# eduardburlacu/DiTSep

Measured on AMD Instinct MI355X. Metric: separated utterances/sec @ N=30, 2-spk 4 s mixtures, higher is better.
Workload: dtype fp16 (fp16 MFMA operands, fp32 accumulate)

## Files before the change

ditsep_amd/csrc/common.h:

```cpp
#pragma once
#include <hip/hip_runtime.h>
#include <stdint.h>

typedef unsigned short op16_t;
typedef __attribute__((ext_vector_type(8))) unsigned short op16x8;
typedef __attribute__((ext_vector_type(4))) unsigned short op16x4;
typedef __attribute__((ext_vector_type(8))) __bf16 bf16x8;
typedef __attribute__((ext_vector_type(8))) _Float16 f16x8;
typedef __attribute__((ext_vector_type(4))) float f32x4;

#define DSN_WAVE 64

#define DSN_PL(planes, f16) ((planes) | ((f16) << 4))
#define PL_COUNT(pl) ((pl)&3)
#define PL_F16(pl) ((pl) >> 4)

enum { DSN_ACT_NONE = 0, DSN_ACT_ELU = 1, DSN_ACT_SNAKE = 2, DSN_ACT_SILU = 3 };
enum { DSN_F32_NONE = 0, DSN_F32_TANH = 1 };

__device__ __forceinline__ float dsn_elu(float v) { return v > 0.f ? v : expm1f(v); }
__device__ __forceinline__ float dsn_silu(float v) { return v / (1.f + __expf(-v)); }
__device__ __forceinline__ float dsn_snake(float v, float alpha, float inv_beta) {
  float s = __sinf(v * alpha);
  return v + inv_beta * s * s;
}

#define DSN_F16_MAX 65504.f
__device__ __forceinline__ float dsn_sat16(float v) {
  const float c = __builtin_amdgcn_fmed3f(v, -DSN_F16_MAX, DSN_F16_MAX);
  return v != v ? v : c;
}
__device__ __forceinline__ op16_t to_op16(float v, int f16) {
  return f16 ? __builtin_bit_cast(unsigned short, (_Float16)dsn_sat16(v)) : __builtin_bit_cast(unsigned short, (__bf16)v);
}
__device__ __forceinline__ float from_op16(op16_t u, int f16) {
  return f16 ? (float)__builtin_bit_cast(_Float16, u) : (float)__builtin_bit_cast(__bf16, u);
}
__device__ __forceinline__ void dsn_split(float v, op16_t& hi, op16_t& lo, int f16) {
  hi = to_op16(v, f16);
  lo = to_op16(v - from_op16(hi, f16), f16);
}

typedef __attribute__((ext_vector_type(8))) int i32x8;
#define DSN_FP8_MAX 448.f
__device__ __forceinline__ int dsn_mx_exp(float amax) {
  const unsigned u = __builtin_bit_cast(unsigned, amax * (1.f / DSN_FP8_MAX));
  const int k = (int)((u >> 23) & 0xffu) - 127 + ((u & 0x7fffffu) ? 1 : 0);
  return min(max(k, -126), 126);
}
__device__ __forceinline__ float dsn_pow2(int k) { return __builtin_bit_cast(float, (unsigned)(127 + k) << 23); }
__device__ __forceinline__ unsigned dsn_fp8x4(const f32x4& v) {
  float c[4];
#pragma unroll
  for (int r = 0; r < 4; ++r) {
    const float m = __builtin_amdgcn_fmed3f(v[r], -DSN_FP8_MAX, DSN_FP8_MAX);
    c[r] = v[r] != v[r] ? v[r] : m;
  }
  int w = __builtin_amdgcn_cvt_pk_fp8_f32(c[0], c[1], 0, false);
  w = __builtin_amdgcn_cvt_pk_fp8_f32(c[2], c[3], w, true);
  return (unsigned)w;
}
__device__ __forceinline__ f32x4 mfma_mx8(const op16x8& w_lo, const op16x8& w_hi, const op16x8& a_lo, const op16x8& a_hi,
                                          const f32x4& c, int sw, int sa) {
  typedef __attribute__((ext_vector_type(4))) int i32x4;
  const i32x4 wl = __builtin_bit_cast(i32x4, w_lo), wh = __builtin_bit_cast(i32x4, w_hi);
  const i32x4 al = __builtin_bit_cast(i32x4, a_lo), ah = __builtin_bit_cast(i32x4, a_hi);
  const i32x8 w = {wl[0], wl[1], wl[2], wl[3], wh[0], wh[1], wh[2], wh[3]};
  const i32x8 a = {al[0], al[1], al[2], al[3], ah[0], ah[1], ah[2], ah[3]};
  return __builtin_amdgcn_mfma_scale_f32_16x16x128_f8f6f4(w, a, c, 0, 0, 0, sw, 0, sa);
}

template <int F16>
__device__ __forceinline__ f32x4 mfma16(const op16x8& w, const op16x8& a, const f32x4& c) {
  if (F16)
    return __builtin_amdgcn_mfma_f32_16x16x32_f16(__builtin_bit_cast(f16x8, w), __builtin_bit_cast(f16x8, a), c, 0, 0, 0);
  else
    return __builtin_amdgcn_mfma_f32_16x16x32_bf16(__builtin_bit_cast(bf16x8, w), __builtin_bit_cast(bf16x8, a), c, 0, 0,
                                                   0);
}

__device__ __forceinline__ float wave_sum(float v) {
#pragma unroll
  for (int o = 32; o > 0; o >>= 1) v += __shfl_xor(v, o, 64);
  return v;
}
__device__ __forceinline__ float wave_max(float v) {
#pragma unroll
  for (int o = 32; o > 0; o >>= 1) v = fmaxf(v, __shfl_xor(v, o, 64));
  return v;
}

struct GnGeom {
  int G, cpg, qpg;
};
__host__ __device__ inline GnGeom gn_geom(int C) {
  const int G = C / 4 < 32 ? C / 4 : 32;
  return GnGeom{G, C / G, C / G / 4};
}
__host__ __device__ inline int gn_tpg(int G, int block) {
  int tpg = 1;
  while (tpg < 64 && G * tpg * 2 <= block) tpg *= 2;
  return tpg;
}
// ... 64 lines not shown
```

ditsep_amd/csrc/igemm.hip:

```cpp
#include "igemm.h"

#ifndef DSN_SETPRIO
#define DSN_SETPRIO 0
#endif

namespace {

constexpr int BM = 128, BN = 128, BK = 32;
constexpr int TILE_ELEMS = 128 * BK;

__device__ __forceinline__ int swz(int row, int chunk) { return chunk ^ ((-(row >> 2)) & 3); }

enum { EPI_STATS = 1, EPI_LNFOLD = 2, EPI_FP8OUT = 4 };
enum { LEAN_NO_DIT = 1, LEAN_NO_NCSN = 2, LEAN_SEEDED = 4 };

template <int NT, int MT>
__device__ __forceinline__ void seed_acc(const GemmDesc& d, f32x4 (&acc)[NT][MT], int mw0, int m_end, int nw0, int lane) {
  const int nq = (lane >> 4) * 4;
#pragma unroll
  for (int tm = 0; tm < MT; ++tm) {
    const int m = mw0 + tm * 16 + (lane & 15);
    const bool mok = m < m_end;
    const int b = mok ? m / d.rows_per_b : 0;
    const int j = mok ? m - b * d.rows_per_b : 0;
// ... 245 lines not shown
  if constexpr ((LEAN & LEAN_SEEDED) == 0 && BIAS_FIRST) {
    if (!f_swiglu) {
#pragma unroll
      for (int tn = 0; tn < NT; ++tn) {
        const int n = nw0 + tn * 16 + nq;
        gbias[tn] = (d.bias && n < d.N) ? *reinterpret_cast<const f32x4*>(d.bias + (n % d.bias_mod)) : f32x4{0.f, 0.f, 0.f, 0.f};
      }
#pragma unroll
      for (int tn = 0; tn < NT; ++tn) dsn_touch(gbias[tn]);
    }
  }
  float gmean[NT], gm2[NT];
#pragma unroll
  for (int tn = 0; tn < NT; ++tn) gmean[tn] = gm2[tn] = 0.f;
#pragma unroll
  for (int tm = 0; tm < MT; ++tm) {
    const int m = mw0 + tm * 16 + (lane & 15);
    if (m >= m_end) continue;
    const int b = m / d.rows_per_b;
    const int j = m - b * d.rows_per_b;
    const long row_rel = (long)j * d.out_row_elems + d.out_off;
    const long row_abs = (long)b * d.out_bstride + row_rel;
    if (!f_swiglu) {
      if (!ROPE_FIRST && f_rope) {
        const int section = nw0 / d.qkv_D;
        if (section < 2 && (nw0 & 63) == 0) {
          const int pos = m % d.rope_S;
          const f32x4 c0 = *reinterpret_cast<const f32x4*>(d.rope_cos + pos * 32 + nq);
          const f32x4 s0 = *reinterpret_cast<const f32x4*>(d.rope_sin + pos * 32 + nq);
          const f32x4 c1 = *reinterpret_cast<const f32x4*>(d.rope_cos + pos * 32 + 16 + nq);
          const f32x4 s1 = *reinterpret_cast<const f32x4*>(d.rope_sin + pos * 32 + 16 + nq);
          const f32x4 x0 = acc[0][tm], x1 = acc[1][tm];
          acc[0][tm] = x0 * c0 - x1 * s0;
          acc[1][tm] = x1 * c1 + x0 * s1;
        }
      }
#pragma unroll
      for (int tn = 0; tn < NT; ++tn) {
        const int n = nw0 + tn * 16 + nq;
        if (n >= d.N) continue;
        const long rel = row_rel + n;
        if (rel < 0 || rel >= d.out_limit) continue;
        const long off = row_abs + n;
        f32x4 v = acc[tn][tm];
        if constexpr ((LEAN & LEAN_SEEDED) == 0) {
          if constexpr (BIAS_FIRST) v += gbias[tn];
          else if (d.bias) v += *reinterpret_cast<const f32x4*>(d.bias + (n % d.bias_mod));
          if (f_qkv && n < d.qkv_D) v *= d.q_scale;
          if (f_bbias) v += *reinterpret_cast<const f32x4*>(d.bbias + (long)b * d.bbias_stride + n);
          if (d.resid)
            v += *reinterpret_cast<const f32x4*>(d.resid + (long)b * d.resid_bstride + (long)j * d.resid_row_elems +
                                                 d.resid_off + n);
        }
        v *= d.out_scale;
        if (f_gn) {
          const float mb = 0.25f * ((v[0] + v[1]) + (v[2] + v[3]));
          float m2b = 0.f;
#pragma unroll
          for (int r = 0; r < 4; ++r) {
            const float dl = v[r] - mb;
            m2b += dl * dl;
          }
          if (tm == 0) {
            gmean[tn] = mb;
            gm2[tn] = m2b;
          } else {
            const float dm = mb - gmean[tn];
            gmean[tn] += dm * (1.f / (float)(tm + 1));
            gm2[tn] += m2b + dm * dm * (4.f * (float)tm / (float)(tm + 1));
          }
        }
        if (d.out_f32) {
          f32x4 o = v;
          if (f_tanh) {
#pragma unroll
            for (int r = 0; r < 4; ++r) o[r] = tanhf(v[r]);
          }
          *reinterpret_cast<f32x4*>(d.out_f32 + off) = o;
        }
        if (d.out_planes) {
          f32x4 a = v;
          if (d.act == DSN_ACT_ELU) {
#pragma unroll
            for (int r = 0; r < 4; ++r) a[r] = dsn_elu(v[r]);
          } else if (d.act == DSN_ACT_SILU) {
#pragma unroll
            for (int r = 0; r < 4; ++r) a[r] = dsn_silu(v[r]);
          } else if (d.act == DSN_ACT_SNAKE) {
            const int ch = n % d.act_mod;
            const f32x4 al = *reinterpret_cast<const f32x4*>(d.act_a + ch);
            const f32x4 ib = *reinterpret_cast<const f32x4*>(d.act_b + ch);
#pragma unroll
            for (int r = 0; r < 4; ++r) a[r] = dsn_snake(v[r], al[r], ib[r]);
          }
          op16x4 hi, lo;
#pragma unroll
          for (int r = 0; r < 4; ++r) {
            op16_t h, l;
            dsn_split(a[r], h, l, F16);
            hi[r] = h;
            lo[r] = l;
          }
          *reinterpret_cast<op16x4*>(d.out_planes + off) = hi;
          if (P == 2) *reinterpret_cast<op16x4*>(d.out_planes + d.out_ps + off) = lo;
        }
      }
    } else if ((EPI & EPI_FP8OUT) && d.out_fp8) {
      static_assert(!(EPI & EPI_FP8OUT) || NT == 4, "fp8 SwiGLU epilogue expects 64 packed columns per wave");
      f32x4 h[2];
      float amax = 0.f;
#pragma unroll
      for (int tp = 0; tp < 2; ++tp) {
        const int np = nw0 + tp * 32;
        f32x4 val = acc[2 * tp][tm], gate = acc[2 * tp + 1][tm];
        if (d.bias && np < d.N) {
          val += *reinterpret_cast<const f32x4*>(d.bias + np + nq);
          gate += *reinterpret_cast<const f32x4*>(d.bias + np + 16 + nq);
        }
#pragma unroll
        for (int r = 0; r < 4; ++r) {
          h[tp][r] = val[r] * dsn_silu(gate[r]);
          amax = fmaxf(amax, fabsf(h[tp][r]));
        }
      }
      amax = fmaxf(amax, __shfl_xor(amax, 16, 64));
      amax = fmaxf(amax, __shfl_xor(amax, 32, 64));
      const int k = dsn_mx_exp(amax);
      const float inv = dsn_pow2(-k);
      if (nw0 < d.N) {
        const long orow = (long)m * (d.N >> 1);
#pragma unroll
        for (int tp = 0; tp < 2; ++tp)
          *reinterpret_cast<unsigned*>(d.out_fp8 + orow + (nw0 >> 1) + tp * 16 + nq) = dsn_fp8x4(h[tp] * inv);
        if ((lane >> 4) == 0) d.out_fp8_scale[(long)m * (d.N >> 6) + (nw0 >> 6)] = (unsigned char)(k + 127);
      }
    } else {
#pragma unroll
      for (int tp = 0; tp < NT / 2; ++tp) {
        const int np = nw0 + tp * 32;
        if (np >= d.N) continue;
        const int feat = (np >> 1) + nq;
        const long off = row_abs + feat;
        f32x4 val = acc[2 * tp][tm], gate = acc[2 * tp + 1][tm];
        if (d.bias) {
          val += *reinterpret_cast<const f32x4*>(d.bias + np + nq);
          gate += *reinterpret_cast<const f32x4*>(d.bias + np + 16 + nq);
        }
        op16x4 hi, lo;
#pragma unroll
        for (int r = 0; r < 4; ++r) {
          op16_t h, l;
          dsn_split(val[r] * dsn_silu(gate[r]), h, l, F16);
          hi[r] = h;
          lo[r] = l;
        }
        *reinterpret_cast<op16x4*>(d.out_planes + off) = hi;
        if (P == 2) *reinterpret_cast<op16x4*>(d.out_planes + d.out_ps + off) = lo;
      }
    }
  }
  if (f_gn && mw0 < m_end) {
    const int b = mw0 / d.rows_per_b;
    const int slice = (mw0 - b * d.rows_per_b) >> 6;
    const int S = d.rows_per_b >> 6;
#pragma unroll
    for (int tn = 0; tn < NT; ++tn) {
      float cnt = (float)(MT * 4);
// ... 1486 lines not shown
```

ditsep_amd/csrc/kernels.hip:

```cpp
#include "kernels.h"

namespace {

constexpr int TPB = 256;
inline int grid_for(long n, int per_block = TPB, int cap = 256 * 16) {
  long g = (n + per_block - 1) / per_block;
  return (int)(g < 1 ? 1 : (g > cap ? cap : g));
}

__device__ __forceinline__ void store_planes(op16_t* dst, long ps, int planes, long i, float v) {
  op16_t h, l;
  dsn_split(v, h, l, PL_F16(planes));
  dst[i] = h;
  if (PL_COUNT(planes) == 2) dst[ps + i] = l;
}

__global__ void pack_tokens_kernel(const float* __restrict__ s0, int C0, const float* __restrict__ s1, int C1,
                                   int B, int T, float* __restrict__ df, op16_t* __restrict__ dp, long ps,
                                   int planes) {
  const int C = C0 + C1;
  const long n = (long)B * T * C;
  for (long i = blockIdx.x * (long)blockDim.x + threadIdx.x; i < n; i += (long)gridDim.x * blockDim.x) {
    const int c = (int)(i % C);
    const long bt = i / C;
// ... 533 lines not shown
                                                             int L, int C, int apply_tanh) {
  constexpr int TILE = 256;
  extern __shared__ __attribute__((aligned(16))) float smem[];
  const int NJ = C / 32;
  f32x4* wl4 = reinterpret_cast<f32x4*>(smem);
  float* part = smem + KT * C;
  const int blocks_per_seq = (L + TILE - 1) / TILE;
  const int s = blockIdx.x / blocks_per_seq;
  const int l0 = (blockIdx.x - s * blocks_per_seq) * TILE;
  const int pad = (KT - 1) / 2;
  for (int i = threadIdx.x; i < KT * C; i += blockDim.x) {
    const int t = i / C, c = i - t * C;
    const int chunk = c >> 3, k = c & 7;
    const int j = chunk >> 2, q = chunk & 3;
    smem[((((t * NJ + j) * 2 + (k >> 2)) * 4 + q) << 2) + (k & 3)] = w[i];
  }
  __syncthreads();
  const int q = threadIdx.x & 3;
  const bool f16 = PL_F16(planes), two = PL_COUNT(planes) == 2;
  for (int r = threadIdx.x >> 2; r < TILE + KT - 1; r += 64) {
    const int l = l0 - pad + r;
    float acc[KT];
#pragma unroll
    for (int t = 0; t < KT; ++t) acc[t] = 0.f;
    if (l >= 0 && l < L) {
      const op16_t* row = a + ((long)s * L + l) * C;
      for (int j = 0; j < NJ; ++j) {
        const int ch = (j * 4 + q) * 8;
        const op16x8 hi = *reinterpret_cast<const op16x8*>(row + ch);
        float v[8];
#pragma unroll
        for (int k = 0; k < 8; ++k) v[k] = from_op16(hi[k], f16);
        if (two) {
          const op16x8 lo = *reinterpret_cast<const op16x8*>(row + ps + ch);
#pragma unroll
          for (int k = 0; k < 8; ++k) v[k] += from_op16(lo[k], f16);
        }
#pragma unroll
        for (int t = 0; t < KT; ++t) {
          const f32x4 wa = wl4[((t * NJ + j) * 2 + 0) * 4 + q], wb = wl4[((t * NJ + j) * 2 + 1) * 4 + q];
          acc[t] += (v[0] * wa[0] + v[1] * wa[1]) + (v[2] * wa[2] + v[3] * wa[3]) + (v[4] * wb[0] + v[5] * wb[1]) +
                    (v[6] * wb[2] + v[7] * wb[3]);
        }
      }
    }
#pragma unroll
    for (int t = 0; t < KT; ++t) {
      float x = acc[t];
      x += __shfl_xor(x, 1, 64);
      x += __shfl_xor(x, 2, 64);
      if (q == 0) part[r * 8 + t] = x;
    }
  }
  __syncthreads();
  for (int p = threadIdx.x; p < TILE; p += blockDim.x) {
    const int l = l0 + p;
    if (l < L) {
      float v = 0.f;
#pragma unroll
      for (int t = 0; t < KT; ++t) v += part[(p + t) * 8 + t];
      out[(long)s * L + l] = apply_tanh ? tanhf(v) : v;
    }
  }
}

__global__ void conv_in1_kernel(const float* __restrict__ wav, const float* __restrict__ w,
                                const float* __restrict__ bias, int L, int Cout, int ktaps,
                                float* __restrict__ of, op16_t* __restrict__ op, long ps, int planes, int act,
                                const float* __restrict__ aa, const float* __restrict__ ab, long total) {
  const int pad = (ktaps - 1) / 2;
  for (long i = blockIdx.x * (long)blockDim.x + threadIdx.x; i < total; i += (long)gridDim.x * blockDim.x) {
    const int co = (int)(i % Cout);
    const long sl = i / Cout;
    const int l = (int)(sl % L);
    const long s = sl / L;
    float acc = bias ? bias[co] : 0.f;
    for (int t = 0; t < ktaps; ++t) {
      const int li = l + t - pad;
      if (li >= 0 && li < L) acc += w[co * ktaps + t] * wav[s * L + li];
    }
    if (of) of[i] = acc;
    if (op) {
      float a = acc;
      if (act == DSN_ACT_ELU) a = dsn_elu(acc);
      else if (act == DSN_ACT_SNAKE) a = dsn_snake(acc, aa[co], ab[co]);
      store_planes(op, ps, planes, i, a);
    }
  }
}

__global__ void conv_in1_vec_kernel(const float* __restrict__ wav, const float* __restrict__ w,
                                    const float* __restrict__ bias, int L, int Cout, int ktaps,
                                    float* __restrict__ of, op16_t* __restrict__ op, long ps, int planes, int act,
                                    const float* __restrict__ aa, const float* __restrict__ ab, long rows) {
  const int cq = Cout >> 2;
  const int c4 = (threadIdx.x % cq) * 4;
  const int pad = (ktaps - 1) / 2;
  float wr[4][8];
  f32x4 bv = {0.f, 0.f, 0.f, 0.f};
#pragma unroll
  for (int r = 0; r < 4; ++r) {
#pragma unroll
    for (int t = 0; t < 8; ++t) wr[r][t] = t < ktaps ? w[(c4 + r) * ktaps + t] : 0.f;
    if (bias) bv[r] = bias[c4 + r];
  }
  const int rpb = blockDim.x / cq;
  for (long row = blockIdx.x * (long)rpb + threadIdx.x / cq; row < rows; row += (long)gridDim.x * rpb) {
    const int l = (int)(row % L);
    const long s = row / L;
    float x[8];
#pragma unroll
    for (int t = 0; t < 8; ++t) {
      const int li = l + t - pad;
      x[t] = (t < ktaps && li >= 0 && li < L) ? wav[s * L + li] : 0.f;
    }
    f32x4 acc = bv;
#pragma unroll
    for (int r = 0; r < 4; ++r)
#pragma unroll
      for (int t = 0; t < 8; ++t) acc[r] += wr[r][t] * x[t];
    const long o = row * Cout + c4;
    if (of) *reinterpret_cast<f32x4*>(of + o) = acc;
    if (op) {
      op16x4 hi, lo;
#pragma unroll
      for (int r = 0; r < 4; ++r) {
        float v = acc[r];
        if (act == DSN_ACT_ELU) v = dsn_elu(v);
        else if (act == DSN_ACT_SNAKE) v = dsn_snake(v, aa[c4 + r], ab[c4 + r]);
        op16_t h, lw;
        dsn_split(v, h, lw, PL_F16(planes));
        hi[r] = h;
        lo[r] = lw;
      }
      *reinterpret_cast<op16x4*>(op + o) = hi;
      if (PL_COUNT(planes) == 2) *reinterpret_cast<op16x4*>(op + ps + o) = lo;
    }
  }
}

__global__ void vae_sample_kernel(const float* __restrict__ enc, const float* __restrict__ noise,
                                  float* __restrict__ y, int D, int T, long total) {
  for (long i = blockIdx.x * (long)blockDim.x + threadIdx.x; i < total; i += (long)gridDim.x * blockDim.x) {
    const int t = (int)(i % T);
    const long sc = i / T;
    const int c = (int)(sc % D);
    const long s = sc / D;
    const float* row = enc + (s * T + t) * (2L * D);
    const float mean = row[c], scale = row[D + c];
    const float sp = scale > 20.f ? scale : log1pf(expf(scale));
    y[i] = noise[i] * (sp + 1e-4f) + mean;
  }
}

__device__ __forceinline__ void philox_round(uint32_t (&c)[4], uint32_t k0, uint32_t k1) {
  const uint64_t p0 = (uint64_t)0xD2511F53u * c[0];
  const uint64_t p1 = (uint64_t)0xCD9E8D57u * c[2];
  const uint32_t n0 = (uint32_t)(p1 >> 32) ^ c[1] ^ k0;
  const uint32_t n1 = (uint32_t)p1;
  const uint32_t n2 = (uint32_t)(p0 >> 32) ^ c[3] ^ k1;
  const uint32_t n3 = (uint32_t)p0;
  c[0] = n0; c[1] = n1; c[2] = n2; c[3] = n3;
}

__global__ void randn_kernel(float* __restrict__ out, long n, unsigned long long seed, unsigned long long offset) {
  const long n4 = (n + 3) >> 2;
  for (long i = blockIdx.x * (long)blockDim.x + threadIdx.x; i < n4; i += (long)gridDim.x * blockDim.x) {
    const unsigned long long ctr = (unsigned long long)i + offset;
    uint32_t c[4] = {(uint32_t)ctr, (uint32_t)(ctr >> 32), 0u, 0u};
    uint32_t k0 = (uint32_t)seed, k1 = (uint32_t)(seed >> 32);
#pragma unroll
    for (int r = 0; r < 10; ++r) {
      philox_round(c, k0, k1);
      k0 += 0x9E3779B9u;
      k1 += 0xBB67AE85u;
    }
    float u[4];
#pragma unroll
    for (int r = 0; r < 4; ++r) u[r] = ((float)(c[r] >> 8) + 0.5f) * (1.0f / 16777216.0f);
    float z[4];
    const float r0 = sqrtf(-2.f * logf(u[0])), r1 = sqrtf(-2.f * logf(u[2]));
    const float tw = 6.283185307179586f;
    z[0] = r0 * cosf(tw * u[1]);
    z[1] = r0 * sinf(tw * u[1]);
    z[2] = r1 * cosf(tw * u[3]);
    z[3] = r1 * sinf(tw * u[3]);
#pragma unroll
    for (int r = 0; r < 4; ++r)
      if (i * 4 + r < n) out[i * 4 + r] = z[r];
  }
}

__global__ void rand_uniform_kernel(float* __restrict__ out, long n, unsigned long long seed,
                                    unsigned long long offset, float lo, float hi) {
  for (long i = blockIdx.x * (long)blockDim.x + threadIdx.x; i < n; i += (long)gridDim.x * blockDim.x) {
    const unsigned long long ctr = (unsigned long long)i + offset;
    uint32_t c[4] = {(uint32_t)ctr, (uint32_t)(ctr >> 32), 0u, 0u};
    uint32_t k0 = (uint32_t)seed, k1 = (uint32_t)(seed >> 32);
#pragma unroll
    for (int r = 0; r < 10; ++r) {
      philox_round(c, k0, k1);
      k0 += 0x9E3779B9u;
      k1 += 0xBB67AE85u;
    }
    const float u = ((float)(c[0] >> 8) + 0.5f) * (1.0f / 16777216.0f);
    out[i] = fminf(lo + (hi - lo) * u, hi);
  }
}

__global__ void wn_scale_kernel(const float* __restrict__ v, const float* __restrict__ g, float* __restrict__ scale,
                                int R, long inner) {
// ... 371 lines not shown
```

ditsep_amd/csrc/ru_fused.hip:

```cpp
#include "igemm.h"
#include "kernels.h"
#include <cstdlib>
#include <functional>

namespace {

constexpr int C = 128;
constexpr int TL = 128;
constexpr int KT = 32;
constexpr int WTILE = 128 * KT;
constexpr int NSTW = 3;

__device__ __forceinline__ int swz32(int row, int chunk) { return chunk ^ ((-(row >> 2)) & 3); }

template <int P, int F16>
__global__ __launch_bounds__(256, 2) void ru_fused_kernel(const RuDesc d, const op16_t* __restrict__ zero_page) {
  extern __shared__ __attribute__((aligned(16))) op16_t lds[];
  const int halo = 3 * d.dil;
  const int hrows = (TL + 2 * halo + 3) & ~3;
  constexpr int AH_ROWS = TL + 54 + 2;
  constexpr int AH_PLANE = AH_ROWS * C;
  op16_t* ah = lds;
  op16_t* ring = lds + P * AH_PLANE;
  constexpr int RING_STAGE = P * WTILE;

  const int tid = threadIdx.x, lane = tid & 63;
  const int wave = __builtin_amdgcn_readfirstlane(tid >> 6);
  const int wm = wave >> 1, wn = wave & 1;
  const int tiles_per_seq = (d.L + TL - 1) / TL;
  const int s = blockIdx.x / tiles_per_seq;
  const int l0 = (blockIdx.x - s * tiles_per_seq) * TL;
  const long seq_off = (long)s * d.L * C;

  {
    const int ninstr = hrows / 4;
    for (int j = wave; j < ninstr; j += 4) {
      const int q = j * 64 + lane;
      const int row = q >> 4, cs = q & 15;
      const int c = (cs - 2 * row) & 15;
      const int l = l0 - halo + row;
      const bool ok = l >= 0 && l < d.L;
#pragma unroll
      for (int p = 0; p < P; ++p) {
        const op16_t* g = ok ? d.A + p * d.a_ps + seq_off + (long)l * C + c * 8 : zero_page + (lane & 3) * 8;
        __builtin_amdgcn_global_load_lds((const __attribute__((address_space(1))) void*)g,
                                         (__attribute__((address_space(3))) void*)(ah + p * AH_PLANE + j * 64 * 8), 16,
                                         0, 0);
      }
    }
  }
  const int rsub = lane >> 2, cpos = lane & 3;
  long wrow_off[2];
#pragma unroll
  for (int gi = 0; gi < 2; ++gi) {
    const int row = (wave * 2 + gi) * 16 + rsub;
    wrow_off[gi] = (long)row * 0 + (cpos ^ swz32(row, 0)) * 8;
  }
  auto issue_w = [&](const op16_t* W, long wps, int ktot, int koff, int stage) {
    op16_t* sb = ring + stage * RING_STAGE;
#pragma unroll
    for (int gi = 0; gi < 2; ++gi) {
      const int row = (wave * 2 + gi) * 16 + rsub;
#pragma unroll
      for (int p = 0; p < P; ++p)
        __builtin_amdgcn_global_load_lds(
            (const __attribute__((address_space(1))) void*)(W + p * wps + (long)row * ktot + koff + wrow_off[gi]),
            (__attribute__((address_space(3))) void*)(sb + p * WTILE + (wave * 2 + gi) * 16 * KT), 16, 0, 0);
    }
  };
  constexpr int G = 2 * P;

  f32x4 acc[4][4];
#pragma unroll
  for (int a = 0; a < 4; ++a)
#pragma unroll
    for (int b = 0; b < 4; ++b) acc[a][b] = f32x4{0.f, 0.f, 0.f, 0.f};

  const int frow = lane & 15, fchunk = lane >> 4;
  const int w_frag = (wn * 64 + frow) * KT + swz32(frow, fchunk) * 8;

  constexpr int NKT7 = 7 * (C / KT);
  issue_w(d.W7, d.w7_ps, 7 * C, 0, 0);
  issue_w(d.W7, d.w7_ps, 7 * C, KT, 1);
  for (int i = 0; i < NKT7; ++i) {
    if (i + 1 < NKT7)
      asm volatile("s_waitcnt vmcnt(%0) lgkmcnt(0)" ::"n"(G) : "memory");
    else
      asm volatile("s_waitcnt vmcnt(0) lgkmcnt(0)" ::: "memory");
    __builtin_amdgcn_s_barrier();
    if (i + 2 < NKT7) issue_w(d.W7, d.w7_ps, 7 * C, (i + 2) * KT, (i + 2) % NSTW);
    const int tap = i >> 2, kc = i & 3;
    const op16_t* wb = ring + (i % NSTW) * RING_STAGE;
    op16x8 fa[P][4], fw[P][4];
#pragma unroll
    for (int p = 0; p < P; ++p)
#pragma unroll
      for (int k = 0; k < 4; ++k) {
        const int row = wm * 64 + k * 16 + frow + tap * d.dil;
        fa[p][k] = *reinterpret_cast<const op16x8*>(ah + p * AH_PLANE + row * C + ((kc * 4 + fchunk + 2 * row) & 15) * 8);
        fw[p][k] = *reinterpret_cast<const op16x8*>(wb + p * WTILE + w_frag + k * 16 * KT);
      }
#pragma unroll
    for (int tn = 0; tn < 4; ++tn)
#pragma unroll
      for (int tm = 0; tm < 4; ++tm) {
        if (P == 2) {
          acc[tn][tm] = mfma16<F16>(fw[P - 1][tn], fa[0][tm], acc[tn][tm]);
          acc[tn][tm] = mfma16<F16>(fw[0][tn], fa[P - 1][tm], acc[tn][tm]);
        }
        acc[tn][tm] = mfma16<F16>(fw[0][tn], fa[0][tm], acc[tn][tm]);
      }
  }
  asm volatile("s_waitcnt lgkmcnt(0)" ::: "memory");
  __builtin_amdgcn_s_barrier();

  issue_w(d.W1, d.w1_ps, C, 0, 0);
  issue_w(d.W1, d.w1_ps, C, KT, 1);
  const int nq = (lane >> 4) * 4;
#pragma unroll
  for (int tm = 0; tm < 4; ++tm) {
    const int m = wm * 64 + tm * 16 + (lane & 15);
#pragma unroll
    for (int tn = 0; tn < 4; ++tn) {
      const int n = wn * 64 + tn * 16 + nq;
      f32x4 v = acc[tn][tm] + *reinterpret_cast<const f32x4*>(d.b7 + n);
      op16x4 hi, lo;
#pragma unroll
      for (int r = 0; r < 4; ++r) {
        float a = v[r];
        if (d.act_mid == DSN_ACT_ELU) a = dsn_elu(a);
        else if (d.act_mid == DSN_ACT_SNAKE) a = dsn_snake(a, d.mid_a[n + r], d.mid_b[n + r]);
        op16_t h, l;
        dsn_split(a, h, l, F16);
        hi[r] = h;
        lo[r] = l;
      }
      const int off = m * C + (((n >> 3) + 2 * m) & 15) * 8 + (n & 7);
      *reinterpret_cast<op16x4*>(ah + off) = hi;
      if (P == 2) *reinterpret_cast<op16x4*>(ah + AH_PLANE + off) = lo;
      acc[tn][tm] = f32x4{0.f, 0.f, 0.f, 0.f};
    }
  }

  constexpr int NKT1 = C / KT;
  for (int i = 0; i < NKT1; ++i) {
    if (i + 1 < NKT1)
      asm volatile("s_waitcnt vmcnt(%0) lgkmcnt(0)" ::"n"(G) : "memory");
    else
      asm volatile("s_waitcnt vmcnt(0) lgkmcnt(0)" ::: "memory");
    __builtin_amdgcn_s_barrier();
    if (i + 2 < NKT1) issue_w(d.W1, d.w1_ps, C, (i + 2) * KT, (i + 2) % NSTW);
    const op16_t* wb = ring + (i % NSTW) * RING_STAGE;
    op16x8 fa[P][4], fw[P][4];
#pragma unroll
    for (int p = 0; p < P; ++p)
#pragma unroll
      for (int k = 0; k < 4; ++k) {
        const int row = wm * 64 + k * 16 + frow;
        fa[p][k] = *reinterpret_cast<const op16x8*>(ah + p * AH_PLANE + row * C + ((i * 4 + fchunk + 2 * row) & 15) * 8);
        fw[p][k] = *reinterpret_cast<const op16x8*>(wb + p * WTILE + w_frag + k * 16 * KT);
      }
#pragma unroll
    for (int tn = 0; tn < 4; ++tn)
#pragma unroll
      for (int tm = 0; tm < 4; ++tm) {
        if (P == 2) {
          acc[tn][tm] = mfma16<F16>(fw[P - 1][tn], fa[0][tm], acc[tn][tm]);
          acc[tn][tm] = mfma16<F16>(fw[0][tn], fa[P - 1][tm], acc[tn][tm]);
        }
        acc[tn][tm] = mfma16<F16>(fw[0][tn], fa[0][tm], acc[tn][tm]);
      }
  }

  f32x4 res[4], nres[4];
  auto load_res = [&](int tm, f32x4 (&r)[4]) {
    const int l = l0 + wm * 64 + tm * 16 + (lane & 15);
    const long rowoff = seq_off + (long)min(l, d.L - 1) * C;
#pragma unroll
    for (int tn = 0; tn < 4; ++tn) r[tn] = *reinterpret_cast<const f32x4*>(d.X + rowoff + wn * 64 + tn * 16 + nq);
  };
  load_res(0, res);
#pragma unroll
  for (int tm = 0; tm < 4; ++tm) {
    if (tm + 1 < 4) load_res(tm + 1, nres);
    const int l = l0 + wm * 64 + tm * 16 + (lane & 15);
    const long rowoff = seq_off + (long)l * C;
#pragma unroll
    for (int tn = 0; tn < 4; ++tn) {
      if (l >= d.L) continue;
      const int n = wn * 64 + tn * 16 + nq;
      f32x4 v = acc[tn][tm] + *reinterpret_cast<const f32x4*>(d.b1 + n) + res[tn];
      if (d.out_f32) *reinterpret_cast<f32x4*>(d.out_f32 + rowoff + n) = v;
      if (d.out_planes) {
        op16x4 hi, lo;
#pragma unroll
        for (int r = 0; r < 4; ++r) {
          float a = v[r];
          if (d.act_out == DSN_ACT_ELU) a = dsn_elu(a);
          else if (d.act_out == DSN_ACT_SNAKE) a = dsn_snake(a, d.out_a[n + r], d.out_b[n + r]);
          op16_t h, lw;
          dsn_split(a, h, lw, F16);
          hi[r] = h;
          lo[r] = lw;
        }
        *reinterpret_cast<op16x4*>(d.out_planes + rowoff + n) = hi;
        if (P == 2) *reinterpret_cast<op16x4*>(d.out_planes + d.out_ps + rowoff + n) = lo;
      }
    }
#pragma unroll
    for (int tn = 0; tn < 4; ++tn) res[tn] = nres[tn];
  }
}

constexpr int TL2 = 256;
constexpr int ACH_ROWS = 384;
constexpr int ACH_STAGE = ACH_ROWS * KT;
constexpr int RING2_OFF = 2 * ACH_STAGE;
constexpr int H_ELEMS = TL2 * C;
constexpr int LDS2_ELEMS = H_ELEMS + 2 * WTILE;

template <int F16>
__global__ __launch_bounds__(512, 4) void ru_fused2_kernel(const RuDesc d, const op16_t* __restrict__ zero_page) {
  extern __shared__ __attribute__((aligned(16))) op16_t lds[];
  const int halo = 3 * d.dil;
  const int tid = threadIdx.x, lane = tid & 63;
  const int wave = __builtin_amdgcn_readfirstlane(tid >> 6);
  const int wm = wave >> 1, wn = wave & 1;
  const int tiles_per_seq = (d.L + TL2 - 1) / TL2;
  const int s = blockIdx.x / tiles_per_seq;
  const int l0 = (blockIdx.x - s * tiles_per_seq) * TL2;
  const long seq_off = (long)s * d.L * C;
  const int nrows = TL2 + 2 * halo;

  const op16_t* a_src[3];
#pragma unroll
  for (int j = 0; j < 3; ++j) {
    const int q = (wave * 3 + j) * 64 + lane;
    const int row = q >> 2, c = (q & 3) ^ ((row >> 1) & 3);
    const int l = l0 - halo + row;
    a_src[j] = (row < nrows && l >= 0 && l < d.L) ? d.A + seq_off + (long)l * C + c * 8 : nullptr;
  }
  auto issue_a = [&](int kc) {
#pragma unroll
    for (int j = 0; j < 3; ++j) {
      const op16_t* g = a_src[j] ? a_src[j] + kc * KT : zero_page + (lane & 3) * 8;
      __builtin_amdgcn_global_load_lds((const __attribute__((address_space(1))) void*)g,
                                       (__attribute__((address_space(3))) void*)(lds + (kc & 1) * ACH_STAGE +
                                                                                  (wave * 3 + j) * 64 * 8),
                                       16, 0, 0);
    }
  };
  const int rsub = lane >> 2, cpos = lane & 3;
  const int wrow = wave * 16 + rsub;
  const int wcol = (cpos ^ swz32(wrow, 0)) * 8;
  auto issue_w = [&](const op16_t* W, int ktot, int koff, op16_t* stage) {
    __builtin_amdgcn_global_load_lds(
        (const __attribute__((address_space(1))) void*)(W + (long)wrow * ktot + koff + wcol),
        (__attribute__((address_space(3))) void*)(stage + wave * 16 * KT), 16, 0, 0);
  };

  f32x4 acc[4][4];
#pragma unroll
  for (int a = 0; a < 4; ++a)
#pragma unroll
    for (int b = 0; b < 4; ++b) acc[a][b] = f32x4{0.f, 0.f, 0.f, 0.f};
  const int frow = lane & 15, fchunk = lane >> 4;
  const int w_frag = (wn * 64 + frow) * KT + swz32(frow, fchunk) * 8;
  op16_t* ring = lds + RING2_OFF;

  issue_a(0);
  issue_w(d.W7, 7 * C, 0, ring);
  issue_w(d.W7, 7 * C, C, ring + WTILE);
  int st = 0;
  for (int kc = 0; kc < 4; ++kc) {
    const op16_t* ach = lds + (kc & 1) * ACH_STAGE;
#pragma unroll
    for (int tap = 0; tap < 7; ++tap) {
      if (kc == 3 && tap == 6)
        asm volatile("s_waitcnt vmcnt(0) lgkmcnt(0)" ::: "memory");
      else if ((tap == 1 || tap == 2) && kc < 3)
        asm volatile("s_waitcnt vmcnt(4) lgkmcnt(0)" ::: "memory");
      else
        asm volatile("s_waitcnt vmcnt(1) lgkmcnt(0)" ::: "memory");
      __builtin_amdgcn_s_barrier();
      {
        int t2 = tap + 2, k2 = kc;
        if (t2 >= 7) { t2 -= 7; ++k2; }
        int s2 = st + 2;
        if (s2 >= NSTW) s2 -= NSTW;
        if (k2 < 4) issue_w(d.W7, 7 * C, t2 * C + k2 * KT, ring + s2 * WTILE);
        if (tap == 0 && kc < 3) issue_a(kc + 1);
      }
      const op16_t* wb = ring + st * WTILE;
      op16x8 fa[4], fw[4];
#pragma unroll
      for (int k = 0; k < 4; ++k) {
        const int row = wm * 64 + k * 16 + frow + tap * d.dil;
        fa[k] = *reinterpret_cast<const op16x8*>(ach + row * KT + ((fchunk ^ ((row >> 1) & 3)) * 8));
        fw[k] = *reinterpret_cast<const op16x8*>(wb + w_frag + k * 16 * KT);
      }
#pragma unroll
      for (int tn = 0; tn < 4; ++tn)
#pragma unroll
        for (int tm = 0; tm < 4; ++tm) acc[tn][tm] = mfma16<F16>(fw[tn], fa[tm], acc[tn][tm]);
      if (++st == NSTW) st = 0;
    }
  }
  asm volatile("s_waitcnt lgkmcnt(0)" ::: "memory");
  __builtin_amdgcn_s_barrier();

  op16_t* ring1 = lds + H_ELEMS;
  issue_w(d.W1, C, 0, ring1);
  issue_w(d.W1, C, KT, ring1 + WTILE);
  const int nq = (lane >> 4) * 4;
#pragma unroll
  for (int tm = 0; tm < 4; ++tm) {
    const int m = wm * 64 + tm * 16 + (lane & 15);
#pragma unroll
    for (int tn = 0; tn < 4; ++tn) {
      const int n = wn * 64 + tn * 16 + nq;
      f32x4 v = acc[tn][tm] + *reinterpret_cast<const f32x4*>(d.b7 + n);
      op16x4 hi;
#pragma unroll
      for (int r = 0; r < 4; ++r) {
        float a = v[r];
        if (d.act_mid == DSN_ACT_ELU) a = dsn_elu(a);
        else if (d.act_mid == DSN_ACT_SNAKE) a = dsn_snake(a, d.mid_a[n + r], d.mid_b[n + r]);
        op16_t h, l;
        dsn_split(a, h, l, F16);
        hi[r] = h;
      }
      *reinterpret_cast<op16x4*>(lds + m * C + (((n >> 3) + 2 * m) & 15) * 8 + (n & 7)) = hi;
      const int ls = l0 + wm * 64 + tm * 16 + (lane & 15);
      acc[tn][tm] = *reinterpret_cast<const f32x4*>(d.b1 + n) +
                    *reinterpret_cast<const f32x4*>(d.X + seq_off + (long)min(ls, d.L - 1) * C + n);
    }
  }

#pragma unroll
  for (int i = 0; i < 4; ++i) {
    if (i == 0)
      asm volatile("s_waitcnt vmcnt(1) lgkmcnt(0)" ::: "memory");
    else
      asm volatile("s_waitcnt vmcnt(0) lgkmcnt(0)" ::: "memory");
    __builtin_amdgcn_s_barrier();
    if (i >= 1 && i + 1 < 4) issue_w(d.W1, C, (i + 1) * KT, ring1 + ((i + 1) & 1) * WTILE);
    const op16_t* wb = ring1 + (i & 1) * WTILE;
    op16x8 fa[4], fw[4];
#pragma unroll
    for (int k = 0; k < 4; ++k) {
      const int row = wm * 64 + k * 16 + frow;
      fa[k] = *reinterpret_cast<const op16x8*>(lds + row * C + ((i * 4 + fchunk + 2 * row) & 15) * 8);
      fw[k] = *reinterpret_cast<const op16x8*>(wb + w_frag + k * 16 * KT);
    }
#pragma unroll
    for (int tn = 0; tn < 4; ++tn)
#pragma unroll
      for (int tm = 0; tm < 4; ++tm) acc[tn][tm] = mfma16<F16>(fw[tn], fa[tm], acc[tn][tm]);
  }

#pragma unroll
  for (int tm = 0; tm < 4; ++tm) {
    const int l = l0 + wm * 64 + tm * 16 + (lane & 15);
    const long rowoff = seq_off + (long)l * C;
#pragma unroll
    for (int tn = 0; tn < 4; ++tn) {
      if (l >= d.L) continue;
      const int n = wn * 64 + tn * 16 + nq;
      const f32x4 v = acc[tn][tm];
      if (d.out_f32) *reinterpret_cast<f32x4*>(d.out_f32 + rowoff + n) = v;
      if (d.out_planes) {
        op16x4 hi;
#pragma unroll
        for (int r = 0; r < 4; ++r) {
          float a = v[r];
          if (d.act_out == DSN_ACT_ELU) a = dsn_elu(a);
          else if (d.act_out == DSN_ACT_SNAKE) a = dsn_snake(a, d.out_a[n + r], d.out_b[n + r]);
          op16_t h, lw;
          dsn_split(a, h, lw, F16);
          hi[r] = h;
        }
        *reinterpret_cast<op16x4*>(d.out_planes + rowoff + n) = hi;
      }
    }
  }
}

const op16_t* ru_zero_page() {
  static op16_t* zp[64] = {};
  op16_t*& z = zp[dsn_current_device()];
  if (!z) {
    if (hipMalloc((void**)&z, 4096) != hipSuccess) return nullptr;
    (void)hipMemset(z, 0, 4096);
  }
  return z;
}

template <int P, int F16>
hipError_t launch_t(const RuDesc& d, hipStream_t st) {
  const op16_t* zp = ru_zero_page();
  if (!zp) return hipErrorOutOfMemory;
  const size_t smem = ((size_t)P * (TL + 56) * C + (size_t)NSTW * P * WTILE) * sizeof(op16_t);
  static std::atomic<unsigned long long> attr{0};
  if (dsn_first_use_on_device(attr)) {
    (void)hipFuncSetAttribute(reinterpret_cast<const void*>(ru_fused_kernel<P, F16>),
                              hipFuncAttributeMaxDynamicSharedMemorySize, 160 * 1024);
  }
  const int grid = d.S * ((d.L + TL - 1) / TL);
  hipLaunchKernelGGL((ru_fused_kernel<P, F16>), dim3(grid), dim3(256), smem, st, d, zp);
  return hipGetLastError();
}

}

template <int F16>
hipError_t launch2_t(const RuDesc& d, hipStream_t st) {
  const op16_t* zp = ru_zero_page();
  if (!zp) return hipErrorOutOfMemory;
  const size_t smem = (size_t)LDS2_ELEMS * sizeof(op16_t);
  static std::atomic<unsigned long long> attr{0};
  if (dsn_first_use_on_device(attr)) {
    (void)hipFuncSetAttribute(reinterpret_cast<const void*>(ru_fused2_kernel<F16>),
                              hipFuncAttributeMaxDynamicSharedMemorySize, 160 * 1024);
  }
  const int grid = d.S * ((d.L + TL2 - 1) / TL2);
  hipLaunchKernelGGL((ru_fused2_kernel<F16>), dim3(grid), dim3(512), smem, st, d, zp);
  return hipGetLastError();
}

static bool ru_act_ok(int kind, const float* a, const float* b) {
  if (kind == DSN_ACT_SNAKE) return a && b;
  return kind == DSN_ACT_NONE || kind == DSN_ACT_ELU;
}

hipError_t ru_fused_launch(const RuDesc& d, int pl, hipStream_t st) {
  if (d.dil < 1 || d.dil > 9 || d.S <= 0 || d.L <= 0) return hipErrorInvalidValue;
  if (!d.A || !d.X || !d.W7 || !d.W1 || !d.b7 || !d.b1 || (!d.out_f32 && !d.out_planes)) return hipErrorInvalidValue;
  if (!ru_act_ok(d.act_mid, d.mid_a, d.mid_b)) return hipErrorInvalidValue;
  if (d.out_planes && !ru_act_ok(d.act_out, d.out_a, d.out_b)) return hipErrorInvalidValue;
  const int P = PL_COUNT(pl), f16 = PL_F16(pl);
  if (d.out_planes) {
    const long n = (long)d.S * d.L * C;
    for (int p = 0; p < P; ++p)
      for (int q = 0; q < P; ++q) {
        const op16_t *a = d.A + p * d.a_ps, *o = d.out_planes + q * d.out_ps;
        if (std::less<const op16_t*>()(a, o + n) && std::less<const op16_t*>()(o, a + n)) return hipErrorInvalidValue;
      }
  }
  const bool v1 = getenv("DSN_RU_V1") != nullptr;
  if (P == 1 && !v1) return f16 ? launch2_t<1>(d, st) : launch2_t<0>(d, st);
  if (P == 1) return f16 ? launch_t<1, 1>(d, st) : launch_t<1, 0>(d, st);
  return f16 ? launch_t<2, 1>(d, st) : launch_t<2, 0>(d, st);
}
```

Baseline: 287.3.

## Specialize fused residual-unit kernel on activations and use cheaper single-plane ELU

Adds a faster ELU for single-plane (fp16/bf16 only) outputs that uses __expf with a Taylor polynomial near zero instead of expm1f, and applies it in the GEMM, direct-conv and fused residual-unit epilogues. The fused2 residual-unit kernel is templated on the mid and out activation kinds, and the output store is specialized on which outputs exist, so per-element runtime branches go away. Pointer arrays are replaced by 32-bit offsets, and lane indices are recomputed behind asm barriers to cut register pressure, with a new L bound check to keep those offsets valid. The cost is more template instantiations and slightly different ELU rounding for negative inputs.

```diff
diff --git a/ditsep_amd/csrc/common.h b/ditsep_amd/csrc/common.h
--- a/ditsep_amd/csrc/common.h
+++ b/ditsep_amd/csrc/common.h
@@ -19,6 +19,17 @@
 enum { DSN_F32_NONE = 0, DSN_F32_TANH = 1 };
 
 __device__ __forceinline__ float dsn_elu(float v) { return v > 0.f ? v : expm1f(v); }
+#define DSN_ELU16_THR 0.0625f
+__device__ __forceinline__ float dsn_elu16(float v) {
+  const float e = __expf(v) - 1.f;
+  const float p = v * fmaf(v, fmaf(v, fmaf(v, 1.f / 24.f, 1.f / 6.f), 0.5f), 1.f);
+  const float neg = fabsf(v) < DSN_ELU16_THR ? p : e;
+  return v > 0.f ? v : neg;
+}
+template <int P>
+__device__ __forceinline__ float dsn_elu_planes(float v) {
+  return P == 1 ? dsn_elu16(v) : dsn_elu(v);
+}
 __device__ __forceinline__ float dsn_silu(float v) { return v / (1.f + __expf(-v)); }
 __device__ __forceinline__ float dsn_snake(float v, float alpha, float inv_beta) {
   float s = __sinf(v * alpha);
diff --git a/ditsep_amd/csrc/igemm.hip b/ditsep_amd/csrc/igemm.hip
--- a/ditsep_amd/csrc/igemm.hip
+++ b/ditsep_amd/csrc/igemm.hip
@@ -351,7 +351,7 @@
           f32x4 a = v;
           if (d.act == DSN_ACT_ELU) {
 #pragma unroll
-            for (int r = 0; r < 4; ++r) a[r] = dsn_elu(v[r]);
+            for (int r = 0; r < 4; ++r) a[r] = dsn_elu_planes<P>(v[r]);
           } else if (d.act == DSN_ACT_SILU) {
 #pragma unroll
             for (int r = 0; r < 4; ++r) a[r] = dsn_silu(v[r]);
diff --git a/ditsep_amd/csrc/kernels.hip b/ditsep_amd/csrc/kernels.hip
--- a/ditsep_amd/csrc/kernels.hip
+++ b/ditsep_amd/csrc/kernels.hip
@@ -639,7 +639,7 @@
     if (of) of[i] = acc;
     if (op) {
       float a = acc;
-      if (act == DSN_ACT_ELU) a = dsn_elu(acc);
+      if (act == DSN_ACT_ELU) a = PL_COUNT(planes) == 1 ? dsn_elu16(acc) : dsn_elu(acc);
       else if (act == DSN_ACT_SNAKE) a = dsn_snake(acc, aa[co], ab[co]);
       store_planes(op, ps, planes, i, a);
     }
@@ -683,7 +683,7 @@
 #pragma unroll
       for (int r = 0; r < 4; ++r) {
         float v = acc[r];
-        if (act == DSN_ACT_ELU) v = dsn_elu(v);
+        if (act == DSN_ACT_ELU) v = PL_COUNT(planes) == 1 ? dsn_elu16(v) : dsn_elu(v);
         else if (act == DSN_ACT_SNAKE) v = dsn_snake(v, aa[c4 + r], ab[c4 + r]);
         op16_t h, lw;
         dsn_split(v, h, lw, PL_F16(planes));
diff --git a/ditsep_amd/csrc/ru_fused.hip b/ditsep_amd/csrc/ru_fused.hip
--- a/ditsep_amd/csrc/ru_fused.hip
+++ b/ditsep_amd/csrc/ru_fused.hip
@@ -1,7 +1,13 @@
 #include "igemm.h"
 #include "kernels.h"
+#include <climits>
 #include <cstdlib>
 #include <functional>
+#include <type_traits>
+
+#ifndef RU_STAMP
+#define RU_STAMP(i)
+#endif
 
 namespace {
 
@@ -128,7 +134,7 @@
 #pragma unroll
       for (int r = 0; r < 4; ++r) {
         float a = v[r];
-        if (d.act_mid == DSN_ACT_ELU) a = dsn_elu(a);
+        if (d.act_mid == DSN_ACT_ELU) a = dsn_elu_planes<P>(a);
         else if (d.act_mid == DSN_ACT_SNAKE) a = dsn_snake(a, d.mid_a[n + r], d.mid_b[n + r]);
         op16_t h, l;
         dsn_split(a, h, l, F16);
@@ -196,7 +202,7 @@
 #pragma unroll
         for (int r = 0; r < 4; ++r) {
           float a = v[r];
-          if (d.act_out == DSN_ACT_ELU) a = dsn_elu(a);
+          if (d.act_out == DSN_ACT_ELU) a = dsn_elu_planes<P>(a);
           else if (d.act_out == DSN_ACT_SNAKE) a = dsn_snake(a, d.out_a[n + r], d.out_b[n + r]);
           op16_t h, lw;
           dsn_split(a, h, lw, F16);
@@ -219,7 +225,14 @@
 constexpr int H_ELEMS = TL2 * C;
 constexpr int LDS2_ELEMS = H_ELEMS + 2 * WTILE;
 
-template <int F16>
+template <int ACT>
+__device__ __forceinline__ float ru_act16(float v, const float* a, const float* b, int ch) {
+  if (ACT == DSN_ACT_ELU) return dsn_elu16(v);
+  if (ACT == DSN_ACT_SNAKE) return dsn_snake(v, a[ch], b[ch]);
+  return v;
+}
+
+template <int F16, int AMID, int AOUT>
 __global__ __launch_bounds__(512, 4) void ru_fused2_kernel(const RuDesc d, const op16_t* __restrict__ zero_page) {
   extern __shared__ __attribute__((aligned(16))) op16_t lds[];
   const int halo = 3 * d.dil;
@@ -232,30 +245,30 @@
   const long seq_off = (long)s * d.L * C;
   const int nrows = TL2 + 2 * halo;
 
-  const op16_t* a_src[3];
+  const op16_t* a_seq = d.A + seq_off;
+  int a_off[3];
 #pragma unroll
   for (int j = 0; j < 3; ++j) {
     const int q = (wave * 3 + j) * 64 + lane;
     const int row = q >> 2, c = (q & 3) ^ ((row >> 1) & 3);
     const int l = l0 - halo + row;
-    a_src[j] = (row < nrows && l >= 0 && l < d.L) ? d.A + seq_off + (long)l * C + c * 8 : nullptr;
+    a_off[j] = (row < nrows && l >= 0 && l < d.L) ? l * C + c * 8 : -1;
   }
   auto issue_a = [&](int kc) {
 #pragma unroll
     for (int j = 0; j < 3; ++j) {
-      const op16_t* g = a_src[j] ? a_src[j] + kc * KT : zero_page + (lane & 3) * 8;
+      const op16_t* g = a_off[j] >= 0 ? a_seq + a_off[j] + kc * KT : zero_page;
       __builtin_amdgcn_global_load_lds((const __attribute__((address_space(1))) void*)g,
                                        (__attribute__((address_space(3))) void*)(lds + (kc & 1) * ACH_STAGE +
                                                                                   (wave * 3 + j) * 64 * 8),
                                        16, 0, 0);
     }
   };
-  const int rsub = lane >> 2, cpos = lane & 3;
-  const int wrow = wave * 16 + rsub;
-  const int wcol = (cpos ^ swz32(wrow, 0)) * 8;
-  auto issue_w = [&](const op16_t* W, int ktot, int koff, op16_t* stage) {
+  auto issue_w = [&](int ln, const op16_t* W, int ktot, int koff, op16_t* stage) {
+    const int wrow = wave * 16 + (ln >> 2);
+    const int wcol = ((ln & 3) ^ swz32(wrow, 0)) * 8;
     __builtin_amdgcn_global_load_lds(
-        (const __attribute__((address_space(1))) void*)(W + (long)wrow * ktot + koff + wcol),
+        (const __attribute__((address_space(1))) void*)(W + (unsigned)(wrow * ktot + koff + wcol)),
         (__attribute__((address_space(3))) void*)(stage + wave * 16 * KT), 16, 0, 0);
   };
 
@@ -268,12 +281,15 @@
   const int w_frag = (wn * 64 + frow) * KT + swz32(frow, fchunk) * 8;
   op16_t* ring = lds + RING2_OFF;
 
+  RU_STAMP(0);
   issue_a(0);
-  issue_w(d.W7, 7 * C, 0, ring);
-  issue_w(d.W7, 7 * C, C, ring + WTILE);
+  issue_w(lane, d.W7, 7 * C, 0, ring);
+  issue_w(lane, d.W7, 7 * C, C, ring + WTILE);
   int st = 0;
   for (int kc = 0; kc < 4; ++kc) {
     const op16_t* ach = lds + (kc & 1) * ACH_STAGE;
+    int frow_kc = wm * 64 + frow;
+    asm volatile("" : "+v"(frow_kc));
 #pragma unroll
     for (int tap = 0; tap < 7; ++tap) {
       if (kc == 3 && tap == 6)
@@ -288,14 +304,14 @@
         if (t2 >= 7) { t2 -= 7; ++k2; }
         int s2 = st + 2;
         if (s2 >= NSTW) s2 -= NSTW;
-        if (k2 < 4) issue_w(d.W7, 7 * C, t2 * C + k2 * KT, ring + s2 * WTILE);
+        if (k2 < 4) issue_w(lane, d.W7, 7 * C, t2 * C + k2 * KT, ring + s2 * WTILE);
         if (tap == 0 && kc < 3) issue_a(kc + 1);
       }
       const op16_t* wb = ring + st * WTILE;
       op16x8 fa[4], fw[4];
 #pragma unroll
       for (int k = 0; k < 4; ++k) {
-        const int row = wm * 64 + k * 16 + frow + tap * d.dil;
+        const int row = frow_kc + k * 16 + tap * d.dil;
         fa[k] = *reinterpret_cast<const op16x8*>(ach + row * KT + ((fchunk ^ ((row >> 1) & 3)) * 8));
         fw[k] = *reinterpret_cast<const op16x8*>(wb + w_frag + k * 16 * KT);
       }
@@ -309,34 +325,34 @@
   asm volatile("s_waitcnt lgkmcnt(0)" ::: "memory");
   __builtin_amdgcn_s_barrier();
 
+  RU_STAMP(1);
   op16_t* ring1 = lds + H_ELEMS;
-  issue_w(d.W1, C, 0, ring1);
-  issue_w(d.W1, C, KT, ring1 + WTILE);
-  const int nq = (lane >> 4) * 4;
+  int lane2 = tid;
+  asm volatile("" : "+v"(lane2));
+  lane2 &= 63;
+  issue_w(lane2, d.W1, C, 0, ring1);
+  issue_w(lane2, d.W1, C, KT, ring1 + WTILE);
+  const int nq = (lane2 >> 4) * 4, mrow = lane2 & 15;
 #pragma unroll
   for (int tm = 0; tm < 4; ++tm) {
-    const int m = wm * 64 + tm * 16 + (lane & 15);
+    const int m = wm * 64 + tm * 16 + mrow;
+    const float *mid_a = d.mid_a, *mid_b = d.mid_b;
+    if (AMID == DSN_ACT_SNAKE) asm volatile("" : "+s"(mid_a), "+s"(mid_b));
 #pragma unroll
     for (int tn = 0; tn < 4; ++tn) {
       const int n = wn * 64 + tn * 16 + nq;
       f32x4 v = acc[tn][tm] + *reinterpret_cast<const f32x4*>(d.b7 + n);
       op16x4 hi;
 #pragma unroll
-      for (int r = 0; r < 4; ++r) {
-        float a = v[r];
-        if (d.act_mid == DSN_ACT_ELU) a = dsn_elu(a);
-        else if (d.act_mid == DSN_ACT_SNAKE) a = dsn_snake(a, d.mid_a[n + r], d.mid_b[n + r]);
-        op16_t h, l;
-        dsn_split(a, h, l, F16);
-        hi[r] = h;
-      }
+      for (int r = 0; r < 4; ++r) hi[r] = to_op16(ru_act16<AMID>(v[r], mid_a, mid_b, n + r), F16);
       *reinterpret_cast<op16x4*>(lds + m * C + (((n >> 3) + 2 * m) & 15) * 8 + (n & 7)) = hi;
-      const int ls = l0 + wm * 64 + tm * 16 + (lane & 15);
+      const int ls = l0 + wm * 64 + tm * 16 + mrow;
       acc[tn][tm] = *reinterpret_cast<const f32x4*>(d.b1 + n) +
                     *reinterpret_cast<const f32x4*>(d.X + seq_off + (long)min(ls, d.L - 1) * C + n);
     }
   }
 
+  RU_STAMP(2);
 #pragma unroll
   for (int i = 0; i < 4; ++i) {
     if (i == 0)
@@ -344,13 +360,13 @@
     else
       asm volatile("s_waitcnt vmcnt(0) lgkmcnt(0)" ::: "memory");
     __builtin_amdgcn_s_barrier();
-    if (i >= 1 && i + 1 < 4) issue_w(d.W1, C, (i + 1) * KT, ring1 + ((i + 1) & 1) * WTILE);
+    if (i >= 1 && i + 1 < 4) issue_w(lane2, d.W1, C, (i + 1) * KT, ring1 + ((i + 1) & 1) * WTILE);
     const op16_t* wb = ring1 + (i & 1) * WTILE;
     op16x8 fa[4], fw[4];
 #pragma unroll
     for (int k = 0; k < 4; ++k) {
-      const int row = wm * 64 + k * 16 + frow;
-      fa[k] = *reinterpret_cast<const op16x8*>(lds + row * C + ((i * 4 + fchunk + 2 * row) & 15) * 8);
+      const int row = wm * 64 + k * 16 + mrow;
+      fa[k] = *reinterpret_cast<const op16x8*>(lds + row * C + ((i * 4 + (lane2 >> 4) + 2 * row) & 15) * 8);
       fw[k] = *reinterpret_cast<const op16x8*>(wb + w_frag + k * 16 * KT);
     }
 #pragma unroll
@@ -359,31 +375,36 @@
       for (int tm = 0; tm < 4; ++tm) acc[tn][tm] = mfma16<F16>(fw[tn], fa[tm], acc[tn][tm]);
   }
 
-#pragma unroll
-  for (int tm = 0; tm < 4; ++tm) {
-    const int l = l0 + wm * 64 + tm * 16 + (lane & 15);
-    const long rowoff = seq_off + (long)l * C;
-#pragma unroll
-    for (int tn = 0; tn < 4; ++tn) {
+  RU_STAMP(3);
+  int lane3 = tid;
+  asm volatile("" : "+v"(lane3));
+  const int mrow_out = lane3 & 15, nq_out = ((lane3 & 63) >> 4) * 4;
+  auto store_out = [&](auto f32_c, auto planes_c) {
+#pragma unroll
+    for (int tm = 0; tm < 4; ++tm) {
+      const int l = l0 + wm * 64 + tm * 16 + mrow_out;
+      const long rowoff = seq_off + (long)l * C;
+      const float *out_a = d.out_a, *out_b = d.out_b;
+      if (AOUT == DSN_ACT_SNAKE) asm volatile("" : "+s"(out_a), "+s"(out_b));
       if (l >= d.L) continue;
-      const int n = wn * 64 + tn * 16 + nq;
-      const f32x4 v = acc[tn][tm];
-      if (d.out_f32) *reinterpret_cast<f32x4*>(d.out_f32 + rowoff + n) = v;
-      if (d.out_planes) {
-        op16x4 hi;
-#pragma unroll
-        for (int r = 0; r < 4; ++r) {
-          float a = v[r];
-          if (d.act_out == DSN_ACT_ELU) a = dsn_elu(a);
-          else if (d.act_out == DSN_ACT_SNAKE) a = dsn_snake(a, d.out_a[n + r], d.out_b[n + r]);
-          op16_t h, lw;
-          dsn_split(a, h, lw, F16);
-          hi[r] = h;
+#pragma unroll
+      for (int tn = 0; tn < 4; ++tn) {
+        const int n = wn * 64 + tn * 16 + nq_out;
+        const f32x4 v = acc[tn][tm];
+        if (decltype(f32_c)::value) *reinterpret_cast<f32x4*>(d.out_f32 + rowoff + n) = v;
+        if (decltype(planes_c)::value) {
+          op16x4 hi;
+#pragma unroll
+          for (int r = 0; r < 4; ++r) hi[r] = to_op16(ru_act16<AOUT>(v[r], out_a, out_b, n + r), F16);
+          *reinterpret_cast<op16x4*>(d.out_planes + rowoff + n) = hi;
         }
-        *reinterpret_cast<op16x4*>(d.out_planes + rowoff + n) = hi;
-      }
-    }
-  }
+      }
+    }
+  };
+  if (d.out_f32 && d.out_planes) store_out(std::true_type{}, std::true_type{});
+  else if (d.out_planes) store_out(std::false_type{}, std::true_type{});
+  else store_out(std::true_type{}, std::false_type{});
+  RU_STAMP(4);
 }
 
 const op16_t* ru_zero_page() {
@@ -413,19 +434,35 @@
 
 }
 
-template <int F16>
+template <int F16, int AMID, int AOUT>
 hipError_t launch2_t(const RuDesc& d, hipStream_t st) {
   const op16_t* zp = ru_zero_page();
   if (!zp) return hipErrorOutOfMemory;
   const size_t smem = (size_t)LDS2_ELEMS * sizeof(op16_t);
   static std::atomic<unsigned long long> attr{0};
   if (dsn_first_use_on_device(attr)) {
-    (void)hipFuncSetAttribute(reinterpret_cast<const void*>(ru_fused2_kernel<F16>),
+    (void)hipFuncSetAttribute(reinterpret_cast<const void*>(ru_fused2_kernel<F16, AMID, AOUT>),
                               hipFuncAttributeMaxDynamicSharedMemorySize, 160 * 1024);
   }
   const int grid = d.S * ((d.L + TL2 - 1) / TL2);
-  hipLaunchKernelGGL((ru_fused2_kernel<F16>), dim3(grid), dim3(512), smem, st, d, zp);
+  hipLaunchKernelGGL((ru_fused2_kernel<F16, AMID, AOUT>), dim3(grid), dim3(512), smem, st, d, zp);
   return hipGetLastError();
+}
+template <int F16, int AMID>
+hipError_t launch2_out(const RuDesc& d, hipStream_t st) {
+  switch (d.out_planes ? d.act_out : DSN_ACT_NONE) {
+    case DSN_ACT_ELU: return launch2_t<F16, AMID, DSN_ACT_ELU>(d, st);
+    case DSN_ACT_SNAKE: return launch2_t<F16, AMID, DSN_ACT_SNAKE>(d, st);
+    default: return launch2_t<F16, AMID, DSN_ACT_NONE>(d, st);
+  }
+}
+template <int F16>
+hipError_t launch2_mid(const RuDesc& d, hipStream_t st) {
+  switch (d.act_mid) {
+    case DSN_ACT_ELU: return launch2_out<F16, DSN_ACT_ELU>(d, st);
+    case DSN_ACT_SNAKE: return launch2_out<F16, DSN_ACT_SNAKE>(d, st);
+    default: return launch2_out<F16, DSN_ACT_NONE>(d, st);
+  }
 }
 
 static bool ru_act_ok(int kind, const float* a, const float* b) {
@@ -434,7 +471,7 @@
 }
 
 hipError_t ru_fused_launch(const RuDesc& d, int pl, hipStream_t st) {
-  if (d.dil < 1 || d.dil > 9 || d.S <= 0 || d.L <= 0) return hipErrorInvalidValue;
+  if (d.dil < 1 || d.dil > 9 || d.S <= 0 || d.L <= 0 || d.L > INT_MAX / C) return hipErrorInvalidValue;
   if (!d.A || !d.X || !d.W7 || !d.W1 || !d.b7 || !d.b1 || (!d.out_f32 && !d.out_planes)) return hipErrorInvalidValue;
   if (!ru_act_ok(d.act_mid, d.mid_a, d.mid_b)) return hipErrorInvalidValue;
   if (d.out_planes && !ru_act_ok(d.act_out, d.out_a, d.out_b)) return hipErrorInvalidValue;
@@ -448,7 +485,7 @@
       }
   }
   const bool v1 = getenv("DSN_RU_V1") != nullptr;
-  if (P == 1 && !v1) return f16 ? launch2_t<1>(d, st) : launch2_t<0>(d, st);
+  if (P == 1 && !v1) return f16 ? launch2_mid<1>(d, st) : launch2_mid<0>(d, st);
   if (P == 1) return f16 ? launch_t<1, 1>(d, st) : launch_t<1, 0>(d, st);
   return f16 ? launch_t<2, 1>(d, st) : launch_t<2, 0>(d, st);
 }
```

New measurement: 289.1 (median of 6 runs). About the same (+0.6%).
